# termuxinator/html5-canvas-raytracer

Hardware: AMD Instinct MI355X
Metric: Mpixel/s (higher is better)
Workload: dtype f64; 1 GPU; cfg3: h8 scene (8 spheres, 2 lights, depth 3, supersample 1) at 3840x2160; SCENE, CAMERA AND LAUNCH TABLE RESIDENT (a static frame rendered again and again: cold_frame / new_camera_every_step are the other cases); one launch per frame; kernel=fma

## Files before the change

html5-canvas-raytracer_amd/csrc/rt_kernel.hip:

```cpp

#include <hip/hip_runtime.h>
#include <math.h>
#include <stdint.h>

#include "rt_device.h"
#include "rt_block.h"
#include "rt_wide.h"

#ifndef RT_STRICT
#define RT_STRICT 0
#endif
#if RT_STRICT
#define RT_LAUNCH_NAME rt_launch_trace_strict
#define RT_SCRATCH_NAME rt_scratch_trace_strict
#else
#define RT_LAUNCH_NAME rt_launch_trace_fast
#define RT_SCRATCH_NAME rt_scratch_trace_fast
#endif

#ifndef RT_WAVES_PER_EU
#define RT_WAVES_PER_EU 2
#endif

constexpr unsigned rt_waves_per_eu(bool refract, bool grid, bool w1) {
// ... 28 lines not shown
  [[maybe_unused]] constexpr uint32_t WG_WAVES = W1 ? 1u : RT_WG_THREADS / 64u;
  constexpr uint32_t KT = W1 ? 64u : RT_WG_THREADS;
  extern __shared__ double lds_raw[];
#if defined(RT_WAVE_LOG) && !RT_STRICT
  if (unsigned long long *const wl = rt_cold_args()->wave_log; wl != nullptr && (threadIdx.x & 63u) == 0u) {
    unsigned long long *q = wl + ((size_t)(blockIdx.z * gridDim.x + blockIdx.x) * WG_WAVES + (threadIdx.x >> 6)) * 4u;
    q[0] = __builtin_amdgcn_s_memrealtime();
    q[2] = (unsigned long long)__builtin_amdgcn_s_getreg((4u) | (0u << 6) | (31u << 11)) | ((unsigned long long)__builtin_amdgcn_s_getreg((20u) | (0u << 6) | (31u << 11)) << 32);
    q[3] = rt_entry_index<W1>();
  }
#endif
  const uint32_t tid = threadIdx.x;
  const uint32_t mtl_words = L.n_objects * (uint32_t)(sizeof(rt_mtl) / 8);
  const uint32_t tex_words = 16u * 2u;
  const bool cull_lds_on = (!RT_STRICT && !COUNT) ? !GRID : (L.cull_in_lds != 0u);
  const uint32_t cull_words = cull_lds_on ? L.n_objects * 4u : 0u;
  constexpr bool MTL_ONLY = W1 && !GRID;
  const uint32_t image_words = MTL_ONLY ? mtl_words : mtl_words + tex_words + cull_words;
  constexpr bool IMAGE_IN_LDS = RT_STRICT || COUNT || !(GRID && !REFRACT);
  const uint32_t lds_words = IMAGE_IN_LDS ? image_words : 0u;
  const double *__restrict__ image = (const double *)L.lds_image;
  typedef uint32_t __attribute__((ext_vector_type(4))) rt_u4;
  constexpr uint32_t RT_STAGE_PIECES = 3u;
  const uint32_t image_vec = image_words >> 1;
  [[maybe_unused]] rt_u4 piece[RT_STAGE_PIECES];
  [[maybe_unused]] double stage0 = 0.0;
  const auto stage_issue = [&](const uint32_t tid) __attribute__((always_inline)) {
    if constexpr (!IMAGE_IN_LDS) {
    } else if constexpr (GRID || W1) {
      const rt_u4 *__restrict__ image4 = (const rt_u4 *)L.lds_image;
#pragma unroll
      for (uint32_t i = 0; i < RT_STAGE_PIECES; i++) if (i * KT < image_vec) piece[i] = image4[tid + i * KT];
    } else {
      stage0 = (tid < image_words) ? image[tid] : 0.0;
    }
  };
  constexpr bool UNI_OK = W1 && !REFRACT && !COUNT && !RT_STRICT && !(GRID && SS2);
  if constexpr (!UNI_OK) stage_issue(tid);
  const rt_mtl *mtl = IMAGE_IN_LDS ? (const rt_mtl *)lds_raw : (const rt_mtl *)L.lds_image;
  const rt_texture_desc *tex = (IMAGE_IN_LDS && !MTL_ONLY) ? (const rt_texture_desc *)(lds_raw + mtl_words) : (const rt_texture_desc *)((const double *)L.lds_image + mtl_words);
  const rt_geom *cull_lds = (const rt_geom *)(lds_raw + mtl_words + tex_words);
  double *acc = lds_raw + lds_words + tid;
  rt_geom cull0 = rt_geom{0.0, 0.0, 0.0, 0.0};
  if (!cull_lds_on) { const uint32_t lane0 = tid & 63u; cull0 = L.cull[lane0 < L.n_loop ? lane0 : 0u]; }

  const uint32_t lane = tid & 63u;
  const rt_pixel P0 = rt_pixel_of<SS2, W1>(L, tid);
#if !RT_STRICT
  if constexpr (W1 && !REFRACT && !COUNT && !GRID) rt_head_batch(L);
  if (P0.rows_valid == 0u) return;
#endif
  [[maybe_unused]] bool uni_try = false;
  [[maybe_unused]] uint32_t cell = 0u;
  if constexpr (UNI_OK) {
    uni_try = !P0.sky && (P0.cand >> 16) == 1u;
    if constexpr (!GRID) cell = (P0.cell >> rt_wave_of<W1>(tid)) & 0x11u;
#ifdef RT_TESTING
    if (L.no_uniform) uni_try = false;
    if (L.no_cells) cell = 0u;
#endif
    if (!uni_try && !P0.sky) stage_issue(tid);
  }
  double rgb[3];
  uint32_t cnt[3] = {0u, 0u, 0u};
  if (P0.sky) {
    rgb[0] = L.sky_rgb[0]; rgb[1] = L.sky_rgb[1]; rgb[2] = L.sky_rgb[2];
  } else {
  const uint32_t px = P0.px, frow = P0.frow, sub = P0.sub;
  const uint32_t sx = SS2 ? 2u * px + (sub & 1u) : px;
  const uint32_t sy = SS2 ? 2u * frow + (sub >> 1) : frow;

#if RT_STRICT
  const double d0 = ((double)sx - L.proj_w) + 0.5, d1 = (L.proj_h - (double)sy) - 0.5, d2 = L.proj_d;
#else
  const double d0 = (double)sx + L.ray_bias[0], d1 = L.ray_bias[1] - (double)sy;
#endif
  const v3 o = mk(L.cam_origin[0], L.cam_origin[1], L.cam_origin[2]);
  double rl;
#if RT_STRICT
  const v3 target = mk(o.x + L.cam_axis_x[0] * d0 + L.cam_axis_y[0] * d0 + L.cam_axis_z[0] * d0,
                       o.y + L.cam_axis_x[1] * d1 + L.cam_axis_y[1] * d1 + L.cam_axis_z[1] * d1,
                       o.z + L.cam_axis_x[2] * d2 + L.cam_axis_y[2] * d2 + L.cam_axis_z[2] * d2);
  const v3 ray = unit(mk(target.x - o.x, target.y - o.y, target.z - o.z), &rl);
#else
  const v3 rawray = mk(L.cam_axis_sum[0] * d0, L.cam_axis_sum[1] * d1, L.ray_bias[2]);
  rl = rt_rsqrt_pos(dot(rawray, rawray));
  const v3 ray = mk(rawray.x * rl, rawray.y * rl, rawray.z * rl);
#endif

#ifdef RT_TESTING
  const bool is_probe = L.probe != nullptr && sx == L.probe_x && sy == L.probe_y && blockIdx.z == 0;
#else
  const bool is_probe = false;
#endif
  const auto stage_finish = [&](const uint32_t tid) __attribute__((always_inline)) {
    if constexpr (!IMAGE_IN_LDS) {
    } else if constexpr (GRID || W1) {
      rt_u4 *lds4 = (rt_u4 *)lds_raw;
      const rt_u4 *__restrict__ image4 = (const rt_u4 *)L.lds_image;
#pragma unroll
      for (uint32_t i = 0; i < RT_STAGE_PIECES; i++) {
        const uint32_t k = tid + i * KT;
        if (i * KT < image_vec && k < image_vec) lds4[k] = piece[i];
      }
      for (uint32_t k = tid + RT_STAGE_PIECES * KT; k < image_vec; k += KT) lds4[k] = image4[k];
    } else {
      if (tid < image_words) lds_raw[tid] = stage0;
      for (uint32_t k = tid + RT_WG_THREADS; k < image_words; k += RT_WG_THREADS) lds_raw[k] = image[k];
    }
  };
  [[maybe_unused]] bool uni_done = false;
  if constexpr (UNI_OK) {
    if (uni_try) {
      uni_done = trace_pixel<REFRACT, COUNT, GRID, SS2, false, W1, true>(L, (const rt_mtl *)L.lds_image, (const rt_texture_desc *)((const double *)L.lds_image + mtl_words), acc,
                                                                         cull_lds, cull0, lane, 0.0, 0.0, 0.0, 0.0, o, ray, rgb, cnt, is_probe, P0.cand | (cell << 24));
      if (!uni_done) {
        uint32_t tid4 = threadIdx.x;
        if constexpr (MTL_ONLY) tid4 = rt_lane_again(); else
        asm volatile("" : "+v"(tid4));
        stage_issue(tid4);
        stage_finish(tid4);
      }
#ifdef RT_TESTING
      else if (lane == 0u && L.uniform_waves != nullptr) {
        atomicAdd(L.uniform_waves, 1ull);
        if (cell & 1u) atomicAdd(L.uniform_waves + 1, 1ull);
      }
#endif
    }
  }
  if (!uni_done) {
    if (!UNI_OK || !uni_try) stage_finish(tid);
    if constexpr (IMAGE_IN_LDS) __syncthreads();

    const double bw = SS2 ? 15.0 : 7.0, bh = SS2 ? 3.0 : 7.0;
    const double lx = SS2 ? (double)(2u * ((lane >> 2) & 7u) + (sub & 1u)) : (double)(lane & 7u);
    const double ly = SS2 ? (double)(2u * (lane >> 5) + (sub >> 1)) : (double)(lane >> 3);
    double blk_x0 = 0.0, blk_x1 = 0.0, blk_y0 = 0.0, blk_y1 = 0.0;
    if (!UNI_OK || !uni_try) { blk_x0 = d0 - lx; blk_x1 = blk_x0 + bw; blk_y1 = d1 + ly; blk_y0 = blk_y1 - bh; }
    trace_pixel<REFRACT, COUNT, GRID, SS2, false, W1>(L, mtl, tex, acc, cull_lds, cull0, lane, blk_x0, blk_x1, blk_y0, blk_y1, o, ray, rgb, cnt, is_probe, P0.cand);
  }
  }

  uint32_t tid2 = threadIdx.x;
  if constexpr (W1 && !GRID) tid2 = rt_lane_again(); else
  asm volatile("" : "+v"(tid2));
  const rt_pixel P1 = rt_pixel_of<SS2, W1>(L, tid2);
#if !RT_STRICT
  const uint32_t wide = rt_cold_args()->wide_stores;
  asm volatile("" :: "s"(wide), "s"(L.scatter), "s"(L.rgb24), "s"(L.w), "s"(L.out), "s"(L.frame_stride));
#endif
  const uint32_t frame_i = blockIdx.z;
  const bool valid = P1.valid;
  const uint32_t r8 = to_byte(rgb[0]), g8 = to_byte(rgb[1]), b8 = to_byte(rgb[2]);
#if RT_STRICT
  uint32_t *__restrict__ out = L.scatter ? L.out_frames[frame_i] : L.out + (size_t)frame_i * L.frame_stride;
  const uint32_t orow = L.scatter ? P1.frow : P1.lrow;
#endif
  uint32_t rgbw;
  if (!SS2) rgbw = r8 | (g8 << 8) | (b8 << 16);
  else {
    uint32_t packed = r8 | (g8 << 10) | (b8 << 20);
    packed += __shfl_xor(packed, 1);
    packed += __shfl_xor(packed, 2);
    rgbw = (((packed & 1023u) + 2u) >> 2) | ((((packed >> 10) & 1023u) + 2u) >> 2 << 8) | ((((packed >> 20) & 1023u) + 2u) >> 2 << 16);
  }
#if RT_STRICT
  const uint32_t n_run = 1u;
#else
  const uint32_t n_run = P1.sky ? P1.run : 1u;
#endif
#if defined(RT_ABLATE_STORE) && !RT_STRICT
  asm volatile("" :: "v"(rgbw));
  const bool store_off = ((RT_ABLATE_STORE + 0) == 2 ? P1.sky : true) && rt_cold_args()->n_frames != ~0u;
#endif
#if !RT_STRICT
  if (wide != 0u) {
    const uint32_t lane2 = tid2 & 63u, wave2 = rt_wave_of<W1>(tid2), pix = rgbw | 0xff000000u;
    const uint32_t px0 = P1.px & ~(RT_TILE_W - 1u);
    uint32_t *const band = L.out + (size_t)frame_i * L.frame_stride + (size_t)(P1.lrow - P1.trow) * L.w;
#if defined(RT_ABLATE_STORE)
    if (store_off) {} else
#endif
    if (P1.sky) {
      const rt_wide_piece wp = rt_wide_sky(lane2);
      const rt_px4 v = {pix, pix, pix, pix};
      for (uint32_t t = wave2; t < n_run; t += 4u) {
        const uint32_t px = px0 + t * RT_TILE_W + wp.col;
        if (wp.row < P1.rows_valid && px < L.w) rt_store16(band + (size_t)wp.row * L.w + px, v, (wide & RT_WIDE_THROUGH_SKY) != 0u);
      }
    } else {
      const rt_wide_piece wp = rt_wide_traced(SS2, wave2, lane2);
      const rt_px4 v = {pix, rt_row_down<SS2 ? 4 : 1>(pix), rt_row_down<SS2 ? 8 : 2>(pix), rt_row_down<SS2 ? 12 : 3>(pix)};
      const uint32_t px = px0 + wp.col;
      if (wp.stores && wp.row < P1.rows_valid && px < L.w) rt_store16(band + (size_t)wp.row * L.w + px, v, (wide & RT_WIDE_THROUGH_TRACED) != 0u);
    }
  } else
#endif
  {
#if !RT_STRICT
  uint32_t *__restrict__ out = L.scatter ? L.out_frames[frame_i] : L.out + (size_t)frame_i * L.frame_stride;
  const uint32_t orow = L.scatter ? P1.frow : P1.lrow;
#endif
  if (!W1 && !L.rgb24 && L.scatter && !SS2) {
    uint32_t *tile = (uint32_t *)(lds_raw + lds_words);
    tile[2u * tid2] = rgbw;
// ... 220 lines not shown
```

html5-canvas-raytracer_amd/csrc/rt_kernel_math.h:

```cpp

struct v3 { double x, y, z; };
__device__ __forceinline__ v3 mk(double x, double y, double z) { v3 r; r.x = x; r.y = y; r.z = z; return r; }
__device__ __forceinline__ double dot(const v3 a, const v3 b) { return a.x * b.x + a.y * b.y + a.z * b.z; }

#if RT_STRICT
__device__ __forceinline__ double rt_sqrt(double x) { return sqrt(x); }
template <bool FMIN = false> __device__ __forceinline__ double rt_sqrt_nn(double x) { return sqrt(x); }
__device__ __forceinline__ double rt_rcp(double x) { return 1.0 / x; }
__device__ __forceinline__ double rt_div(double a, double b) { return a / b; }
__device__ __forceinline__ double rt_pow(double x, double e) { return pow(x, e); }
#define RT_DIV_CONST(x, c) ((x) / (c))
__device__ __forceinline__ v3 unit(const v3 v, double *len_out) {
  const double l = sqrt(dot(v, v));
  *len_out = l;
  if (l != 0.0) { const double s = 1.0 / l; return mk(v.x * s, v.y * s, v.z * s); }
  return v;
}
#else
__device__ __forceinline__ double rt_rsqrt_pos(double m) {
  const double y = __builtin_amdgcn_rsq(m);
  const double e = __builtin_fma(-(m * y), y, 1.0);
  return __builtin_fma(0.5 * y, e, y);
}
__device__ __forceinline__ double rt_sqrt(double x) {
  const double y = rt_rsqrt_pos(x);
  double g = x * y;
  g = __builtin_fma(__builtin_fma(-g, g, x), 0.5 * y, g);
  return (x > 0.0) ? g : x;
}
template <bool FMIN = false>
__device__ __forceinline__ double rt_sqrt_nn(double x) {
  double y;
  if constexpr (FMIN) y = __builtin_fmin(__builtin_amdgcn_rsq(x), 1e100);
  else {
    const unsigned long long yb = __builtin_bit_cast(unsigned long long, __builtin_amdgcn_rsq(x));
    const int32_t yh = (int32_t)(yb >> 32);
    y = __builtin_bit_cast(double, ((unsigned long long)(uint32_t)(yh < 0x7fe00000 ? yh : 0x7fe00000) << 32) | (uint32_t)yb);
  }
  const double e = __builtin_fma(-(x * y), y, 1.0);
  y = __builtin_fma(0.5 * y, e, y);
  const double g = x * y;
  return __builtin_fma(__builtin_fma(-g, g, x), 0.5 * y, g);
}
__device__ __forceinline__ double rt_rcp(double x) {
  double y = __builtin_amdgcn_rcp(x);
  y = __builtin_fma(y, __builtin_fma(-x, y, 1.0), y);
  return __builtin_fma(y, __builtin_fma(-x, y, 1.0), y);
}
__device__ __forceinline__ double rt_div(double a, double b) {
  const double r = rt_rcp(b);
  const double q = a * r;
  return __builtin_fma(__builtin_fma(-q, b, a), r, q);
}
#define RT_DIV_CONST(x, c) rt_div_const((x), (c), 1.0 / (c))
__device__ __forceinline__ double rt_div_const(double a, double c, double rc) {
  const double q = a * rc;
  return __builtin_fma(__builtin_fma(-q, c, a), rc, q);
}
__device__ __attribute__((noinline)) double rt_pow_generic(double x, double e) { return pow(x, e); }
template <bool UNI = false, class EP>
__device__ __forceinline__ double rt_pow_spec(double x, int32_t n, EP e) {
  const int32_t n0 = UNI ? n : __builtin_amdgcn_readfirstlane(n);
  if (UNI || __ballot(n != n0) == 0ull) {
    if (n0 < 0) return rt_pow_generic(x, *e);
    uint32_t k = (uint32_t)n0;
    if (k == 0u) return 1.0;
    double b = x;
    uint32_t g = __builtin_ctz(k);
    for (uint32_t i = 0; i < g; i++) b *= b;
    double r = b;
    for (k >>= g + 1u; k != 0u; k >>= g + 1u) {
      g = __builtin_ctz(k);
      for (uint32_t i = 0; i <= g; i++) b *= b;
      r *= b;
    }
    return r;
  }
  if (n < 0) return rt_pow_generic(x, *e);
  double r = 1.0, b = x;
  uint32_t k = (uint32_t)n;
  do { if (k & 1u) r *= b; b *= b; k >>= 1; } while (__ballot(k != 0u) != 0ull);
  return r;
}
__device__ __forceinline__ v3 unit(const v3 v, double *len_out) {
  const double m = dot(v, v);
  const double s = rt_rsqrt_pos(m);
  const bool ok = (m > 0.0);
  *len_out = ok ? m * s : m;
  return ok ? mk(v.x * s, v.y * s, v.z * s) : v;
}
#endif

#if RT_STRICT
#include "rt_fdlibm.h"
template <bool FMIN = false> __device__ __forceinline__ void rt_atan2_asin(double y, double x, double w, double *at, double *as) { *at = fd_atan2(y, x); *as = fd_asin(w); }
#else
__device__ __forceinline__ double rt_fma_k(double a, double b, double k) {
  double r;
  asm("v_fma_f64 %0, %1, %2, %3" : "=v"(r) : "v"(a), "v"(b), "s"(k));
  return r;
}
typedef const double __attribute__((address_space(4))) *rt_trig_kptr;
typedef double __attribute__((ext_vector_type(4))) rt_d4;
#define RT_TRIG_AHEAD 2u
__constant__ unsigned long long RT_TRIG_BITS[32] = {
    0x3eeba404b5e68a13ull, 0xbf23e260bd3237f4ull, 0x3f4b2bb069efb384ull, 0xbf67952daf56de9bull,
    0x3f7d6d43a595c56full, 0xbf8c6ea4a57d9582ull, 0x3f967e295f08b19full, 0xbf9e9ae6fc27006aull,
    0x3fa2c15b5711927aull, 0x3fa059859fea6a70ull, 0xbfa59976e82d3ff0ull, 0xbf90a5a378a05eafull,
    0x3fa82d5d6ef28734ull, 0x3f94052137024d6aull, 0xbfaae5ce6a214619ull, 0x3f7ab3a098a70509ull,
    0x3fae1bb48427b883ull, 0x3f88ed60a300c8d2ull, 0xbfb110e48b207f05ull, 0x3f8c6fa84b77012bull,
    0x3fb3b13657b87036ull, 0x3f91c6c111dccb70ull, 0xbfb745d119378e4full, 0x3f96e89f0a0adacfull,
    0x3fbc71c717e1913cull, 0x3f9f1c72c668963full, 0xbfc2492492376b7dull, 0x3fa6db6db41ce4bdull,
    0x3fc99999999952ccull, 0x3fb333333336fd5bull, 0xbfd5555555555523ull, 0x3fc5555555555380ull};
template <bool FMIN = false>
__device__ __forceinline__ void rt_atan2_asin(double y, double x, double w, double *at, double *as) {
  rt_trig_kptr K = (rt_trig_kptr)(const void *)RT_TRIG_BITS;
  asm volatile("" : "+s"(K));
#define RT_TRIG_GROUP(I) (*(const rt_d4 __attribute__((address_space(4))) *)(K + 4 * (I)))
  rt_d4 g[8];
  g[0] = RT_TRIG_GROUP(0); g[1] = RT_TRIG_GROUP(1);
  const double ax = __builtin_fabs(x), ay = __builtin_fabs(y);
  const double hi = __builtin_fmax(ax, ay), lo = __builtin_fmin(ax, ay);
  const double q = rt_div(lo, hi);
  const double z = q * q;
  const double yw = __builtin_fabs(w);
  const double t = __builtin_fma(yw, -0.5, 0.5);
  const bool big = (yw >= 0.5);
  const double r = big ? t : w * w;
  g[2] = RT_TRIG_GROUP(2);
  double p = g[0][0];
  p = rt_fma_k(p, z, g[0][1]); p = rt_fma_k(p, z, g[0][2]); p = rt_fma_k(p, z, g[0][3]);
  g[3] = RT_TRIG_GROUP(3);
  p = rt_fma_k(p, z, g[1][0]); p = rt_fma_k(p, z, g[1][1]); p = rt_fma_k(p, z, g[1][2]); p = rt_fma_k(p, z, g[1][3]);
  double pa = 0.0;
#pragma unroll
// ... 67 lines not shown
```

html5-canvas-raytracer_amd/csrc/rt_kernel_trace.h:

```cpp

#define RT_PIN() asm volatile("")
#define RT_ROOT(TCA, DISC)                                                                    \
        const double thc_ = rt_sqrt_nn<REFRACT>(DISC);                                                 \
        const double t0_ = (TCA) - thc_, t1_ = (TCA) + thc_;                                  \
        const bool in_ = (t0_ < eps);                                                         \
        const double t_ = in_ ? t1_ : t0_;
#define RT_CAND(IDX, TCA, DISC)                                                               \
      if (!((DISC) < 0.0)) {                                                                  \
        RT_PIN();                                                                             \
        RT_ROOT(TCA, DISC)                                                                    \
        const bool closer_ = (t_ < ht) && !(t_ < eps);              \
        ht = closer_ ? t_ : ht;                                                               \
        hcode = closer_ ? ((int)(2u * (IDX)) + (in_ ? 1 : 0)) : hcode;                        \
      }
#define RT_GENERIC(IDX, G)                                                                    \
      {                                                                                       \
        const v3 Lv_ = mk((G).ox - p.x, (G).oy - p.y, (G).oz - p.z);                          \
        const double tca_ = dot(d, Lv_);                                                      \
        const double disc_ = (G).r2 - (dot(Lv_, Lv_) - tca_ * tca_);                          \
        RT_CAND(IDX, tca_, disc_)                                                             \
      }
#define RT_ANCHORED_DISC(G)                                                                   \
        const double tca_ = d.x * (G).ox + d.y * (G).oy + d.z * (G).oz;                       \
        const double disc_ = __builtin_fma(tca_, tca_, -(G).r2);
#define RT_ANCHORED(IDX, G)                                                                   \
      {                                                                                       \
        RT_ANCHORED_DISC(G)                                                                   \
        RT_CAND(IDX, tca_, disc_)                                                             \
      }

#if !RT_STRICT
__device__ __forceinline__ float rt_q_of(float qp, float x, float c, float rp_over_r) {
  const float ic = __builtin_amdgcn_rcpf(fmaxf(c, 1e-30f));
  return fminf(ic * (qp * (6.f * x + rp_over_r) + x + 0.5f * x * x) + x, 1e30f);
}
__device__ __forceinline__ int rt_lvl(int lv) { return lv & 255; }
#define RT_Q_GET(L_) __builtin_bit_cast(float, (uint32_t)(L_) & 0xffff0000u)
__device__ __forceinline__ int rt_q_put(int lv, float q) { return (int)(((uint32_t)lv & 0xffffu) | ((__builtin_bit_cast(uint32_t, q) + 0xffffu) & 0xffff0000u)); }
__device__ __forceinline__ float rt_r_get(int lv) { return __builtin_bit_cast(float, ((uint32_t)lv & 0xff00u) << 15); }
__device__ __forceinline__ int rt_r_put(int lv, float r) { return (int)(((uint32_t)lv & 0xffff00ffu) | ((((__builtin_bit_cast(uint32_t, r) >> 23) + 1u) & 255u) << 8)); }
constexpr float RT_Q_FLAT = 4096.f;
#define RT_Q_OF(QP, T, INVR, C, RP) rt_q_of((QP), (T) * (INVR), (C), (RP) * (INVR))
#else
__device__ __forceinline__ int rt_lvl(int lv) { return lv; }
#endif

#if !RT_STRICT
#define RT_XY_INDEX(XU, XV, FU, FV)                                                                                \
          const unsigned long long su = __builtin_bit_cast(unsigned long long, (XU) + 6442450944.0), sv = __builtin_bit_cast(unsigned long long, (XV) + 6442450944.0);   \
          uint32_t iu = __builtin_amdgcn_alignbit((uint32_t)(su >> 32), (uint32_t)su, 20u) ^ 0x80000000u;        \
          uint32_t iv = __builtin_amdgcn_alignbit((uint32_t)(sv >> 32), (uint32_t)sv, 20u) ^ 0x80000000u;       \
           \
// ... 10 lines not shown
              const float ex = (float)(h.x - K->cam_origin[0]), ey = (float)(h.y - K->cam_origin[1]), ez = (float)(h.z - K->cam_origin[2]);   \
              q_here = RT_Q_OF(0.f, __builtin_sqrtf(ex * ex + ey * ey + ez * ez), (float)m.inv_r, __builtin_fabsf((float)dot(d, n)), 0.f);       \
            }                                                                                                     \
            double tol = (K->mark_flags & RT_MARK_ALL) ? 2.0 : K->flag_tol * (double)fmaxf(1.f, q_here * (1.f / RT_Q_FLAT));   \
                          \
            if ((K->mark_flags & (RT_MARK_WEIGHT | RT_MARK_ALL)) == RT_MARK_WEIGHT) {                              \
              double S_ = map_valid ? acc[0] : 1.0;                                                               \
              if constexpr (FOLD_FORWARD && REFRACT) for (int i_ = 0; i_ < sp; i_++) S_ *= (parked[i_].map_valid ? parked[i_].S : 1.0) * parked[i_].a3;   \
              if (__builtin_fabs(S_) * 510.0 < 0.9) tol = -1.0;                                                    \
            }                                                                                                     \
             \
            const bool zf = !(K->mark_flags & RT_MARK_ZERO);                                                       \
            const bool bu = (zf && (FU) == 0.0 && (XU) == 0.0) || (__builtin_fabs((XU) - __builtin_rint(XU)) >= tol);    \
            const bool bv = (zf && (FV) == 0.0 && (XV) == 0.0) || (__builtin_fabs((XV) - __builtin_rint(XV)) >= tol);    \
            if (!(bu & bv)) {                                                                                      \
              uint32_t t3 = threadIdx.x;                                                                          \
              if constexpr (W1 && !GRID) t3 = rt_lane_again(); else                                               \
              asm volatile("" : "+v"(t3));                                                                        \
              rt_mark_append<SS2>(rt_pixel_of<SS2, W1>(L, t3));                                                        \
            }                                                                                                     \
          }
#endif

#if !RT_STRICT
#define RT_SDISC(G, TC, DISC)                                                                 \
            const double TC = -(sv.x * (G).ox + sv.y * (G).oy + sv.z * (G).oz);               \
            const double DISC = __builtin_fma(TC, TC, -(G).r2);
#define RT_SROOTS(TC, THC, T0, T1) const double T0 = llen - (TC + THC), T1 = llen - (TC - THC);
#else
#define RT_SDISC(G, TC, DISC)                                                                 \
            const v3 Lv_ = mk((G).ox - h.x, (G).oy - h.y, (G).oz - h.z);                      \
            const double TC = dot(sv, Lv_);                                                   \
            const double DISC = (G).r2 - (dot(Lv_, Lv_) - TC * TC);
#define RT_SROOTS(TC, THC, T0, T1) const double T0 = TC - THC, T1 = TC + THC;
#endif
#define RT_SHADOW(J, G)                                                                       \
            {                                                                                 \
              const bool other_ = ((int)(J) != hi);                                           \
              if (COUNT && other_ && !blocked) tests++;                                       \
              RT_SDISC(G, tc_, disc_)                                                         \
              if (other_ && !(disc_ < 0.0) && !blocked) {                                     \
                RT_PIN();                                                                     \
                const double thc_ = rt_sqrt_nn<REFRACT>(disc_);                                        \
                RT_SROOTS(tc_, thc_, t0_, t1_)                                                \
                const double t_ = (t0_ < eps) ? t1_ : t0_;                                    \
                if ((t_ < llen) && !(t_ < eps)) {                                             \
                  RT_PIN();                                                                   \
                  const double oa4_ = objs[J].albedo[4];                                      \
                  if (oa4_ != 0.0) li = rt_div(li, oa4_);    \
                  else { li = 0.0; blocked = true; }                                          \
                }                                                                             \
              }                                                                               \
            }
#define RT_SHADOW_U(J, G)                                                                     \
            {                                                                               \
              RT_SDISC(G, tc_, disc_)                                                       \
              if (((int)(J) != hi) && !(disc_ < 0.0)) {                                     \
                RT_PIN();                                                                   \
                const double thc_ = rt_sqrt_nn<REFRACT>(disc_);                                      \
                RT_SROOTS(tc_, thc_, t0_, t1_)                                              \
                const double t_ = (t0_ < eps) ? t1_ : t0_;                                  \
                if ((t_ < llen) && !(t_ < eps) && li != 0.0) {                              \
                  RT_PIN();                                                                 \
                  const double oa4_ = objs[J].albedo[4];                                    \
                  li = (oa4_ != 0.0) ? rt_div(li, oa4_) : 0.0;                              \
                }                                                                           \
              }                                                                             \
            }

#define RT_CHAIN_END()                                                                                                          \
        if constexpr (SIX_WAVES) {                                                                                              \
          if (map_valid) {                                                                                                      \
            const double S_ = acc[0];                                                                                           \
            _Pragma("unroll")                                                                                                   \
            for (int c = 0; c < 3; c++) ret[c] = rt_max_nn(acc[(4 + c) * 64u], rt_min_nn(acc[(7 + c) * 64u], __builtin_fma(S_, ret[c], acc[(1 + c) * 64u])));   \
          }                                                                                                                     \
        }

template <bool REFRACT, bool COUNT, bool GRID, bool SS2, bool ITEM = false, bool W1 = false, bool UNI = false>
__device__ __forceinline__ bool trace_pixel(const rt_launch &L, const rt_mtl *mtl, const rt_texture_desc *tex,
                                            [[maybe_unused]] double *acc, [[maybe_unused]] const rt_geom *cull_lds, [[maybe_unused]] const rt_geom cull0, [[maybe_unused]] uint32_t lane,
                                            [[maybe_unused]] double blk_x0, [[maybe_unused]] double blk_x1, [[maybe_unused]] double blk_y0,
                                            [[maybe_unused]] double blk_y1, v3 p, v3 d, double rgb[3], uint32_t cnt[3],
                                            [[maybe_unused]] bool is_probe, [[maybe_unused]] uint32_t cand_host,
                                            [[maybe_unused]] uint32_t own_sx = 0u, [[maybe_unused]] uint32_t own_sy = 0u, [[maybe_unused]] uint32_t own_f = 0u) {
  static_assert(!UNI || (W1 && !REFRACT && !COUNT && !ITEM && !RT_STRICT), "uniform-material path: the one-wave-workgroup product kernels");
#ifdef RT_TESTING
  uint32_t probe_n = 0;
  double probe_li = 0.0;
#endif
  const sphere_kptr objs = (sphere_kptr)L.objects;
  const geom_kptr geom = (geom_kptr)L.geom;
  const uint32_t N = L.n_objects, NL = L.n_lights;
  const double eps = L.epsilon;
  const uint32_t NLOOP = L.n_loop;
  const uint32_t enc = L.enclosing;
  const bool cull_lds_on = (!RT_STRICT && !COUNT) ? (!GRID && !W1) : (L.cull_in_lds != 0u);
#if RT_STRICT
  constexpr bool FOLD_FORWARD = false;
#else
  constexpr bool FOLD_FORWARD = true;
#endif
  constexpr bool LEAN = !RT_STRICT && !REFRACT && !COUNT && !ITEM;
  [[maybe_unused]] frame<REFRACT> stack[FOLD_FORWARD ? 1 : RT_MAX_SEGS];
  [[maybe_unused]] park parked[(FOLD_FORWARD && REFRACT) ? RT_MAX_SEGS : 1];
  [[maybe_unused]] int sp = 0;
  [[maybe_unused]] bool map_valid = false;
  int level = 0;
  [[maybe_unused]] uint32_t tree_path = 1u;
#if defined(RT_TESTING) && defined(RT_ABLATE_BOUNCE)
  uint32_t segs_left = L.segs ? 1 : 0;
#else
  uint32_t segs_left = L.segs;
#endif
  double ret[3] = {0.0, 0.0, 0.0};
  constexpr bool SIX_WAVES = FOLD_FORWARD && W1 && !GRID && !REFRACT && !COUNT && !ITEM && !UNI;
  constexpr bool WAVE_NODE = LEAN && !GRID && !UNI;
  [[maybe_unused]] uint32_t turn = 0u;

  double ht = RT_INF; int hcode = -1;
  if constexpr (UNI) { if (segs_left == 0) return false; }
  if (segs_left != 0) {
        [[maybe_unused]] const geom_kptr ga = (geom_kptr)L.geom_cam;
#if !RT_STRICT
        if constexpr (UNI) {
          const uint32_t i = cand_host & 255u;
          const rt_geom g0 = rt_load_geom32(ga, i);
          typename rt_mtl_src<true>::type &mu = *rt_mtl_at<true>(mtl, i);
          if ((mu.albedo[3] > 0.0 && segs_left > 1) || rt_mtl_kind(mu) == RT_SAMPLER_STARS) return false;
          RT_ANCHORED_DISC(g0)
          const double t0_ = tca_ - rt_sqrt_nn<REFRACT>(disc_);
          const bool met_ = !(disc_ < 0.0) && (t0_ < ht) && !(t0_ < eps);
          if (__ballot(!met_) != 0ull) return false;
#if defined(RT_TESTING) && defined(RT_ABLATE_UNIFORM)
          rgb[0] = rgb[1] = rgb[2] = 0.0;
          return true;
#endif
          ht = t0_; hcode = (int)(2u * i);
        } else
        if (cand_host != 0u) {
          { const uint32_t i = cand_host & 255u; const rt_geom g0 = rt_load_geom32(ga, i); RT_ANCHORED(i, g0) }
          if (cand_host >= (2u << 16)) { const uint32_t i = (cand_host >> 8) & 255u; const rt_geom g0 = rt_load_geom32(ga, i); RT_ANCHORED(i, g0) }
        } else
#endif
        for (uint32_t base = 0; base < NLOOP; base += 64u) {
          const uint32_t j = base + lane;
          const uint32_t jj = j < NLOOP ? j : 0u;
          double c0 = cull0.ox, c1 = cull0.oy, c2 = cull0.oz, c3 = cull0.r2;
          if constexpr (ITEM) {
          } else if (cull_lds_on) {
            const rt_geom __attribute__((address_space(3))) *g = (const rt_geom __attribute__((address_space(3))) *)cull_lds + jj;
            c0 = g->ox; c1 = g->oy; c2 = g->oz; c3 = g->r2;
          } else if (base != 0u || (W1 && !GRID)) {
            const rt_geom __attribute__((address_space(1))) *g = (const rt_geom __attribute__((address_space(1))) *)L.cull + jj;
            c0 = g->ox; c1 = g->oy; c2 = g->oz; c3 = g->r2;
          }
// ... 223 lines not shown
          col[0] = RT_DIV_CONST((double)(texel & 255u), 255.0); col[1] = RT_DIV_CONST((double)((texel >> 8) & 255u), 255.0);
          col[2] = RT_DIV_CONST((double)((texel >> 16) & 255u), 255.0);
        } else if (kind == RT_SAMPLER_CHECKER) {
          if constexpr (!UNI) rt_atan2_asin<REFRACT>(-n.y, -n.x, -n.z, &t_at, &t_as);
          const double u = RT_DIV_CONST(t_at, M_PI) / 2.0 + 0.5;
          const double v = RT_DIV_CONST(t_as, M_PI / 2.0) / 2.0 + 0.5;
          const double xu = u * m.c[6], xv = v * m.c[7];
          RT_XY_INDEX(xu, xv, m.c[6], m.c[7])
          const int c = (int)((iu ^ iv) & 1u);
          if constexpr (UNI) {
            double k0 = m.c[0], k1 = m.c[1], k2 = m.c[2], k3 = m.c[3], k4 = m.c[4], k5 = m.c[5];
            asm volatile("" : "+s"(k0), "+s"(k1), "+s"(k2), "+s"(k3), "+s"(k4), "+s"(k5));
            col[0] = c ? k3 : k0; col[1] = c ? k4 : k1; col[2] = c ? k5 : k2;
          } else { col[0] = m.c[3 * c]; col[1] = m.c[3 * c + 1]; col[2] = m.c[3 * c + 2]; }
#endif
        } else if (!UNI && kind == RT_SAMPLER_STARS) {
          uint32_t sx = own_sx, sy = own_sy, f = own_f;
          if constexpr (!ITEM) {
            f = blockIdx.z;
            uint32_t t3 = threadIdx.x;
            if constexpr (W1 && !GRID) t3 = rt_lane_again(); else
            asm volatile("" : "+v"(t3));
            const rt_pixel P = rt_pixel_of<SS2, W1>(L, t3);
            sx = SS2 ? 2u * P.px + (P.sub & 1u) : P.px; sy = SS2 ? 2u * P.frow + (P.sub >> 1) : P.frow;
          }
          const unsigned long long pix = (unsigned long long)sy * (SS2 ? 2u * L.w : L.w) + sx;
          const uint32_t path = REFRACT ? tree_path : (1u << rt_lvl(level));
          const rt_launch __attribute__((address_space(4))) *K = rt_cold_args();
          const uint32_t mix = lowbias32(K->stars_seed + K->stars_step * f);
          double c = star_uniform((uint32_t)pix, (uint32_t)(pix >> 32), path, mix);
          c = (c >= m.c[6]) ? 0.0 : c * m.c[7];
          col[0] = col[1] = col[2] = c;
        } else { col[0] = m.c[0]; col[1] = m.c[1]; col[2] = m.c[2]; }
#if !RT_STRICT
        }
#endif

        if constexpr (FOLD_FORWARD && REFRACT) {
#pragma unroll
          for (int c = 0; c < 3; c++) acc[(10 + c) * RT_WG_THREADS] = col[c];
        }

        double diffuse = 0.0, specular = 0.0;
        [[maybe_unused]] double draw = 0.0, sraw = 0.0;
#if defined(RT_TESTING) && defined(RT_ABLATE_LIGHT)
        if (false) {
#else
        if (a1 > 0.0 || a2 > 0.0) {
#endif
          double li = RT_COLD(light_intensity);
#if !RT_STRICT
          [[maybe_unused]] uint32_t smask = ~0u;
          if constexpr (!COUNT) { if (primary_node) smask = rt_entry_shadow_masks<W1>(L); }
#endif
          for (uint32_t k = 0; k < NL; k++) {
            double llen;
            const double *lk = (const double *)((const char *)&L.lights[0][0] + (uint32_t)(k * 24u));
#if !RT_STRICT
            [[maybe_unused]] rt_geom_pair gp_first;
            if constexpr (!GRID && !COUNT) {
              [[maybe_unused]] const geom_kptr gl = (geom_kptr)L.geom_light;
              gp_first = rt_load_geom_pair32(gl, k * L.n_objects);
            }
#endif
            const v3 sraw = mk(lk[0] - h.x, lk[1] - h.y, lk[2] - h.z);
            const double lmag = dot(sraw, sraw);
#if RT_STRICT
            const v3 sv = unit(sraw, &llen);
#else
            const double inv_llen = rt_rsqrt_pos(lmag);
            llen = lmag * inv_llen;
            const v3 sv = mk(sraw.x * inv_llen, sraw.y * inv_llen, sraw.z * inv_llen);
#endif
            const double sdot = dot(sv, l);
#if RT_STRICT
            if (sdot <= 0.0) continue;
#else
            if (!(sdot > 0.0)) continue;
#endif
            if (COUNT) cnt[1]++;
            uint32_t tests = 0;
            bool blocked = false;
#if !RT_STRICT
            const geom_kptr gl = (geom_kptr)L.geom_light;
            const uint32_t glo = k * L.n_objects;
#else
            const geom_kptr gl = geom;
            const uint32_t glo = 0u;
#endif
#if defined(RT_TESTING) && defined(RT_ABLATE_SHADOW)
            const uint32_t NS = 0;
#elif defined(RT_TESTING) && defined(RT_ABLATE_SHADOW4)
            const uint32_t NS = NLOOP > 4u ? NLOOP - 4u : NLOOP;
#else
            const uint32_t NS = NLOOP;
#endif
#if !RT_STRICT
            bool no_occluder = false;
            if constexpr (!COUNT) no_occluder = primary_node && k < 2u && ((smask >> (16u * k)) & 0xffffu) == 0u;
            if (no_occluder) {
            } else
            if (GRID && rt_cold_args()->shadow_grid != nullptr && li != 0.0) {
              const void *const sgrid = rt_cold_args()->shadow_grid;
              const double __attribute__((address_space(4))) *gh = (const double __attribute__((address_space(4))) *)sgrid + 16u * k;
              const v3 vv = mk(-sraw.x, -sraw.y, -sraw.z);
              const double vx = gh[0] * vv.x + gh[1] * vv.y + gh[2] * vv.z, vy = gh[3] * vv.x + gh[4] * vv.y + gh[5] * vv.z;
              const double vz = gh[6] * vv.x + gh[7] * vv.y + gh[8] * vv.z;
              const double iz = rt_rcp(vz);
              const double fx = __builtin_fmin(__builtin_fmax((vx * iz - gh[9]) * gh[11], 0.0), (double)(RT_SGRID - 1));
              const double fy = __builtin_fmin(__builtin_fmax((vy * iz - gh[10]) * gh[12], 0.0), (double)(RT_SGRID - 1));
              const bool proj = (vz > 0.0) && (fx == fx) && (fy == fy);
              const uint32_t cell = proj ? (uint32_t)fy * RT_SGRID + (uint32_t)fx : (uint32_t)(RT_SGRID * RT_SGRID);
              const uint32_t words = (NLOOP + 63u) >> 6;
              const uint32_t cells_at = 16u * NL + k * (RT_SGRID * RT_SGRID + 1u) * words;
              for (uint32_t wd = 0; wd < words; wd++) {
                unsigned long long cand = 0ull, todo = __ballot(true);
                while (todo) {
                  const uint32_t c0 = (uint32_t)__builtin_amdgcn_readlane((int)cell, (int)__builtin_ctzll(todo));
                  cand |= rt_load_word32(sgrid, cells_at + c0 * words + wd);
                  todo &= ~__ballot(cell == c0);
                }
                while (cand) {
                  const uint32_t j = (wd << 6) + (uint32_t)__builtin_ctzll(cand);
                  cand &= cand - 1ull;
                  const rt_geom g0 = rt_load_geom32(gl, glo + j);
                  RT_SHADOW_U(j, g0)
                }
              }
            } else
#endif
            if (!COUNT) {
              if constexpr (UNI) RT_PIN();
              if (li != 0.0) {
                uint32_t j = 0;
#if !RT_STRICT
                [[maybe_unused]] uint32_t mk = ~0u;
                if constexpr (!GRID) { if (primary_node && k < 2u) mk = (smask >> (16u * k)) | 0xffff0000u; }
                if constexpr (!GRID) {
                  if (NS >= 2u) { if (mk & 3u) { const rt_geom g0 = gp_first.a, g1 = gp_first.b; RT_SHADOW_U(0u, g0) RT_SHADOW_U(1u, g1) } j = 2u; }
                }
#endif
                for (; j + 2 <= NS; j += 2) {
#if !RT_STRICT
                  if constexpr (WAVE_NODE) { if (((mk >> (j < 30u ? j : 30u)) & 3u) == 0u) continue; } else
                  if (!GRID && j < 31u && ((mk >> j) & 3u) == 0u) continue;
#endif
                  const rt_geom_pair gp = rt_load_geom_pair32(gl, glo + j);
                  const rt_geom g0 = gp.a, g1 = gp.b;
                  RT_SHADOW_U(j, g0) RT_SHADOW_U(j + 1, g1)
                }
#if !RT_STRICT
                if (j < NS && (GRID || j >= 32u || ((mk >> j) & 1u))) { const rt_geom g0 = rt_load_geom32(gl, glo + j); RT_SHADOW_U(j, g0) }
#else
                if (j < NS) { const rt_geom g0 = rt_load_geom32(gl, glo + j); RT_SHADOW_U(j, g0) }
#endif
              }
            } else
            if (COUNT || li != 0.0) {
              uint32_t j = 0;
              for (; j + 2 <= NS; j += 2) {
                const rt_geom g0 = rt_load_geom32(gl, glo + j), g1 = rt_load_geom32(gl, glo + j + 1);
                RT_SHADOW(j, g0) RT_SHADOW(j + 1, g1)
                if (blocked) break;
              }
              if (j < NS && !blocked) { const rt_geom g0 = rt_load_geom32(gl, glo + j); RT_SHADOW(j, g0) }
            }
            if (COUNT) cnt[2] += tests;
            if (li == 0.0) continue;
#if RT_STRICT
            diffuse += li * sdot / lmag;
#else
            diffuse += (li * sdot) * (inv_llen * inv_llen);
#endif
#if defined(RT_TESTING) && defined(RT_ABLATE_SPEC)
            if (false) {
#else
            if (a2 > 0.0) {
#endif
#if RT_STRICT
              double ql;
              const v3 q = unit(reflect(mk(-sv.x, -sv.y, -sv.z), l), &ql);
              const double spd = d.x * -q.x + d.y * -q.y + d.z * -q.z;
#else
              const double t2 = 2.0 * sdot;
              const v3 q = mk(__builtin_fma(l.x, t2, -sv.x), __builtin_fma(l.y, t2, -sv.y), __builtin_fma(l.z, t2, -sv.z));
              const double spd = -(d.x * q.x + d.y * q.y + d.z * q.z);
#endif
#if !RT_STRICT
              typename rt_mtl_src<UNI>::type *spec_m = &m;
              if constexpr (GRID && !REFRACT && !COUNT && !UNI) {
                uint32_t off_ = (uint32_t)hi * (uint32_t)sizeof(rt_mtl);
                asm volatile("" : "+v"(off_));
                spec_m = (const rt_mtl *)((const char *)mtl + off_);
              }
              const int32_t spec_n = spec_m->spec_n;
              if (spd > 0.0) specular += rt_pow_spec<UNI>(spd, spec_n, &spec_m->specular_exponent);
#else
              if (spd > 0.0) specular += rt_pow(spd, m.specular_exponent);
#endif
            }
          }
          if constexpr (UNI) {
            draw = diffuse; sraw = specular;
            diffuse = rt_min1_nn(diffuse) * a1;
            specular = rt_min1_nn(specular) * a2;
          } else {
          diffuse = min1(diffuse) * a1;
          specular = min1(specular) * a2;
          }
#ifdef RT_TESTING
          probe_li = li;
#endif
        }

        if constexpr (SIX_WAVES) {
          uint32_t hi2 = (uint32_t)hi;
          asm volatile("" : "+v"(hi2));
          const rt_mtl &m2 = *rt_mtl_at<false>(mtl, hi2);
          a0 = m2.albedo[0]; a3 = m2.albedo[3];
        }

#if RT_STRICT
        const v3 nq = n;
#else
        const v3 nq = inside ? mk(-l.x, -l.y, -l.z) : l;
#endif
        v3 r = mk(0, 0, 0); double rlen = 0.0;
#if !RT_STRICT
        if constexpr (LEAN) { if (!UNI && a3 > 0.0 && segs_left > 1) r = unit_go(reflect(d, l), &rlen); } else
#endif
        if (!UNI && a3 > 0.0 && segs_left > 1) r = unit(reflect(d, nq), &rlen);
        v3 f = mk(0, 0, 0); double flen = 0.0;
        if (REFRACT && a4 > 0.0 && segs_left > 1) {
          const double dn = dot(d, nq);
          double cosi = -((dn < -1.0) ? -1.0 : min1(dn));
          v3 nn = nq; double eta;
          if (cosi < 0.0) { cosi = -cosi; nn = mk(-nq.x, -nq.y, -nq.z); eta = m.refract_index; }
          else eta = rt_rcp(m.refract_index);
          const double k = 1.0 - eta * eta * (1.0 - cosi * cosi);
          if (k > 0.0) {
            const double q = eta * cosi - rt_sqrt(k);
            f = mk(d.x * eta + nn.x * q, d.y * eta + nn.y * q, d.z * eta + nn.z * q);
          } else f = reflect(d, nn);
          f = unit(f, &flen);
        }

        if constexpr (FOLD_FORWARD && REFRACT) {
#pragma unroll
          for (int c = 0; c < 3; c++) col[c] = acc[(10 + c) * RT_WG_THREADS];
// ... 195 lines not shown
```

Measured before the change: 171,400 Mpixel/s.

## Keep wave-uniform flags and shadow masks in scalar registers, ladder spec pow

Packs the per-wave sky and uniform-try decisions into one flag word pinned to scalar registers. The sky colour is now filled in at store time, so the sky and uniform paths branch on scalar conditions instead of vector masks. In the uniform, non-grid, single-wave path, shadow occluder masks and the albedo nonzero test also go through scalar values, and the specular integer power uses an unrolled compile-time ladder instead of a gap loop. The aim is fewer VCC/exec-mask branches and fewer VGPRs; in exchange the code is larger and relies on inline-asm pinning, and a census script is added to count branch types in the assembly listing.

```diff
diff --git a/html5-canvas-raytracer_amd/csrc/rt_kernel.hip b/html5-canvas-raytracer_amd/csrc/rt_kernel.hip
--- a/html5-canvas-raytracer_amd/csrc/rt_kernel.hip
+++ b/html5-canvas-raytracer_amd/csrc/rt_kernel.hip
@@ -104,6 +104,23 @@
 #endif
   [[maybe_unused]] bool uni_try = false;
   [[maybe_unused]] uint32_t cell = 0u;
+  constexpr bool WAVE_FLAGS = UNI_OK && !GRID;
+  [[maybe_unused]] uint32_t wf = 0u;
+  if constexpr (WAVE_FLAGS) {
+    cell = (P0.cell >> rt_wave_of<W1>(tid)) & 0x11u;
+#ifdef RT_TESTING
+    if (L.no_cells) cell = 0u;
+#endif
+    if (P0.sky) wf = 2u;
+    else {
+      if ((P0.cand >> 16) == 1u) wf = 1u;
+#ifdef RT_TESTING
+      if (L.no_uniform) wf = 0u;
+#endif
+      if ((wf & 1u) == 0u) stage_issue(tid);
+    }
+    asm volatile("" : "+s"(wf));
+  } else
   if constexpr (UNI_OK) {
     uni_try = !P0.sky && (P0.cand >> 16) == 1u;
     if constexpr (!GRID) cell = (P0.cell >> rt_wave_of<W1>(tid)) & 0x11u;
@@ -113,11 +130,13 @@
 #endif
     if (!uni_try && !P0.sky) stage_issue(tid);
   }
+  const auto wf_bit0 = [&]() __attribute__((always_inline)) { uint32_t w_ = wf; asm volatile("" : "+s"(w_)); return (w_ & 1u) != 0u; };
+#define RT_UNI_TRY() (WAVE_FLAGS ? wf_bit0() : uni_try)
   double rgb[3];
   uint32_t cnt[3] = {0u, 0u, 0u};
-  if (P0.sky) {
+  if (!WAVE_FLAGS && P0.sky) {
     rgb[0] = L.sky_rgb[0]; rgb[1] = L.sky_rgb[1]; rgb[2] = L.sky_rgb[2];
-  } else {
+  } else if (!WAVE_FLAGS || (wf & 2u) == 0u) {
   const uint32_t px = P0.px, frow = P0.frow, sub = P0.sub;
   const uint32_t sx = SS2 ? 2u * px + (sub & 1u) : px;
   const uint32_t sy = SS2 ? 2u * frow + (sub >> 1) : frow;
@@ -163,7 +182,7 @@
   };
   [[maybe_unused]] bool uni_done = false;
   if constexpr (UNI_OK) {
-    if (uni_try) {
+    if (RT_UNI_TRY()) {
       uni_done = trace_pixel<REFRACT, COUNT, GRID, SS2, false, W1, true>(L, (const rt_mtl *)L.lds_image, (const rt_texture_desc *)((const double *)L.lds_image + mtl_words), acc,
                                                                          cull_lds, cull0, lane, 0.0, 0.0, 0.0, 0.0, o, ray, rgb, cnt, is_probe, P0.cand | (cell << 24));
       if (!uni_done) {
@@ -182,17 +201,18 @@
     }
   }
   if (!uni_done) {
-    if (!UNI_OK || !uni_try) stage_finish(tid);
+    if (!UNI_OK || !RT_UNI_TRY()) stage_finish(tid);
     if constexpr (IMAGE_IN_LDS) __syncthreads();
 
     const double bw = SS2 ? 15.0 : 7.0, bh = SS2 ? 3.0 : 7.0;
     const double lx = SS2 ? (double)(2u * ((lane >> 2) & 7u) + (sub & 1u)) : (double)(lane & 7u);
     const double ly = SS2 ? (double)(2u * (lane >> 5) + (sub >> 1)) : (double)(lane >> 3);
     double blk_x0 = 0.0, blk_x1 = 0.0, blk_y0 = 0.0, blk_y1 = 0.0;
-    if (!UNI_OK || !uni_try) { blk_x0 = d0 - lx; blk_x1 = blk_x0 + bw; blk_y1 = d1 + ly; blk_y0 = blk_y1 - bh; }
+    if (!UNI_OK || !RT_UNI_TRY()) { blk_x0 = d0 - lx; blk_x1 = blk_x0 + bw; blk_y1 = d1 + ly; blk_y0 = blk_y1 - bh; }
     trace_pixel<REFRACT, COUNT, GRID, SS2, false, W1>(L, mtl, tex, acc, cull_lds, cull0, lane, blk_x0, blk_x1, blk_y0, blk_y1, o, ray, rgb, cnt, is_probe, P0.cand);
   }
   }
+#undef RT_UNI_TRY
 
   uint32_t tid2 = threadIdx.x;
   if constexpr (W1 && !GRID) tid2 = rt_lane_again(); else
@@ -204,6 +224,7 @@
 #endif
   const uint32_t frame_i = blockIdx.z;
   const bool valid = P1.valid;
+  if constexpr (WAVE_FLAGS) { if (P1.sky) { rgb[0] = L.sky_rgb[0]; rgb[1] = L.sky_rgb[1]; rgb[2] = L.sky_rgb[2]; } }
   const uint32_t r8 = to_byte(rgb[0]), g8 = to_byte(rgb[1]), b8 = to_byte(rgb[2]);
 #if RT_STRICT
   uint32_t *__restrict__ out = L.scatter ? L.out_frames[frame_i] : L.out + (size_t)frame_i * L.frame_stride;
diff --git a/html5-canvas-raytracer_amd/csrc/rt_kernel_math.h b/html5-canvas-raytracer_amd/csrc/rt_kernel_math.h
--- a/html5-canvas-raytracer_amd/csrc/rt_kernel_math.h
+++ b/html5-canvas-raytracer_amd/csrc/rt_kernel_math.h
@@ -58,29 +58,21 @@
   return __builtin_fma(__builtin_fma(-q, c, a), rc, q);
 }
 __device__ __attribute__((noinline)) double rt_pow_generic(double x, double e) { return pow(x, e); }
-template <bool UNI = false, class EP>
+#include "rt_spec_walk.h"
+#define RT_SPEC_LADDER 9
+template <bool UNI = false, bool LADDER = false, class EP>
 __device__ __forceinline__ double rt_pow_spec(double x, int32_t n, EP e) {
+  const auto mul = [](double a, double b) __attribute__((always_inline)) { return a * b; };
   const int32_t n0 = UNI ? n : __builtin_amdgcn_readfirstlane(n);
   if (UNI || __ballot(n != n0) == 0ull) {
     if (n0 < 0) return rt_pow_generic(x, *e);
-    uint32_t k = (uint32_t)n0;
+    const uint32_t k = (uint32_t)n0;
     if (k == 0u) return 1.0;
-    double b = x;
-    uint32_t g = __builtin_ctz(k);
-    for (uint32_t i = 0; i < g; i++) b *= b;
-    double r = b;
-    for (k >>= g + 1u; k != 0u; k >>= g + 1u) {
-      g = __builtin_ctz(k);
-      for (uint32_t i = 0; i <= g; i++) b *= b;
-      r *= b;
-    }
-    return r;
+    if constexpr (LADDER) return rt_spec_walk_ladder<RT_SPEC_LADDER>(k, x, mul);
+    else return rt_spec_walk_gaps(k, x, mul);
   }
   if (n < 0) return rt_pow_generic(x, *e);
-  double r = 1.0, b = x;
-  uint32_t k = (uint32_t)n;
-  do { if (k & 1u) r *= b; b *= b; k >>= 1; } while (__ballot(k != 0u) != 0ull);
-  return r;
+  return rt_spec_walk_lanes((uint32_t)n, x, mul, [](bool more) __attribute__((always_inline)) { return __ballot(more) != 0ull; });
 }
 __device__ __forceinline__ v3 unit(const v3 v, double *len_out) {
   const double m = dot(v, v);
diff --git a/html5-canvas-raytracer_amd/csrc/rt_kernel_trace.h b/html5-canvas-raytracer_amd/csrc/rt_kernel_trace.h
--- a/html5-canvas-raytracer_amd/csrc/rt_kernel_trace.h
+++ b/html5-canvas-raytracer_amd/csrc/rt_kernel_trace.h
@@ -1,3 +1,5 @@
+
+#include "rt_uniform_pred.h"
 
 #define RT_PIN() asm volatile("")
 #define RT_ROOT(TCA, DISC)                                                                    \
@@ -114,6 +116,12 @@
                 }                                                                             \
               }                                                                               \
             }
+__device__ __forceinline__ bool rt_nonzero_scalar(double x) {
+  unsigned long long b_ = __builtin_bit_cast(unsigned long long, x);
+  asm volatile("" : "+s"(b_));
+  return rt_nonzero_bits(b_);
+}
+#define RT_OA4_NONZERO(X) (SIX_FORMS ? rt_nonzero_scalar(X) : ((X) != 0.0))
 #define RT_SHADOW_U(J, G)                                                                     \
             {                                                                               \
               RT_SDISC(G, tc_, disc_)                                                       \
@@ -125,7 +133,7 @@
                 if ((t_ < llen) && !(t_ < eps) && li != 0.0) {                              \
                   RT_PIN();                                                                 \
                   const double oa4_ = objs[J].albedo[4];                                    \
-                  li = (oa4_ != 0.0) ? rt_div(li, oa4_) : 0.0;                              \
+                  li = RT_OA4_NONZERO(oa4_) ? rt_div(li, oa4_) : 0.0;                       \
                 }                                                                           \
               }                                                                             \
             }
@@ -164,6 +172,7 @@
   constexpr bool FOLD_FORWARD = true;
 #endif
   constexpr bool LEAN = !RT_STRICT && !REFRACT && !COUNT && !ITEM;
+  [[maybe_unused]] constexpr bool SIX_FORMS = LEAN && W1 && !GRID;
   [[maybe_unused]] frame<REFRACT> stack[FOLD_FORWARD ? 1 : RT_MAX_SEGS];
   [[maybe_unused]] park parked[(FOLD_FORWARD && REFRACT) ? RT_MAX_SEGS : 1];
   [[maybe_unused]] int sp = 0;
@@ -493,6 +502,7 @@
 #if !RT_STRICT
           [[maybe_unused]] uint32_t smask = ~0u;
           if constexpr (!COUNT) { if (primary_node) smask = rt_entry_shadow_masks<W1>(L); }
+          [[maybe_unused]] const unsigned long long smask64 = 0xffffffff00000000ull | smask;
 #endif
           for (uint32_t k = 0; k < NL; k++) {
             double llen;
@@ -538,6 +548,12 @@
 #endif
 #if !RT_STRICT
             bool no_occluder = false;
+            [[maybe_unused]] uint32_t occ = ~0u;
+            if constexpr (SIX_FORMS) {
+              occ = (uint32_t)(smask64 >> (16u * (k < 2u ? k : 2u)));
+              if constexpr (UNI) asm volatile("" : "+s"(occ));
+              no_occluder = (occ & 0xffffu) == 0u;
+            } else
             if constexpr (!COUNT) no_occluder = primary_node && k < 2u && ((smask >> (16u * k)) & 0xffffu) == 0u;
             if (no_occluder) {
             } else
@@ -576,6 +592,8 @@
                 uint32_t j = 0;
 #if !RT_STRICT
                 [[maybe_unused]] uint32_t mk = ~0u;
+                if constexpr (SIX_FORMS) mk = occ | 0xffff0000u;
+                else
                 if constexpr (!GRID) { if (primary_node && k < 2u) mk = (smask >> (16u * k)) | 0xffff0000u; }
                 if constexpr (!GRID) {
                   if (NS >= 2u) { if (mk & 3u) { const rt_geom g0 = gp_first.a, g1 = gp_first.b; RT_SHADOW_U(0u, g0) RT_SHADOW_U(1u, g1) } j = 2u; }
@@ -583,7 +601,7 @@
 #endif
                 for (; j + 2 <= NS; j += 2) {
 #if !RT_STRICT
-                  if constexpr (WAVE_NODE) { if (((mk >> (j < 30u ? j : 30u)) & 3u) == 0u) continue; } else
+                  if constexpr (WAVE_NODE || (UNI && !GRID)) { if (((mk >> (j < 30u ? j : 30u)) & 3u) == 0u) continue; } else
                   if (!GRID && j < 31u && ((mk >> j) & 3u) == 0u) continue;
 #endif
                   const rt_geom_pair gp = rt_load_geom_pair32(gl, glo + j);
@@ -635,7 +653,7 @@
                 spec_m = (const rt_mtl *)((const char *)mtl + off_);
               }
               const int32_t spec_n = spec_m->spec_n;
-              if (spd > 0.0) specular += rt_pow_spec<UNI>(spd, spec_n, &spec_m->specular_exponent);
+              if (spd > 0.0) specular += rt_pow_spec<UNI, SIX_FORMS>(spd, spec_n, &spec_m->specular_exponent);
 #else
               if (spd > 0.0) specular += rt_pow(spd, m.specular_exponent);
 #endif
diff --git a/html5-canvas-raytracer_amd/csrc/rt_spec_walk.h b/html5-canvas-raytracer_amd/csrc/rt_spec_walk.h
--- /dev/null
+++ b/html5-canvas-raytracer_amd/csrc/rt_spec_walk.h
@@ -0,0 +1,64 @@
+#ifndef RT_SPEC_WALK_H
+#define RT_SPEC_WALK_H
+
+#include <stdint.h>
+
+#ifndef RT_SPEC_WALK_FN
+#if defined(__HIPCC__)
+#define RT_SPEC_WALK_FN __device__ __forceinline__
+#else
+#define RT_SPEC_WALK_FN static inline
+#endif
+#endif
+
+template <class MUL>
+RT_SPEC_WALK_FN double rt_spec_walk_gaps(uint32_t k, double x, MUL mul) {
+  double b = x;
+  uint32_t g = (uint32_t)__builtin_ctz(k);
+  for (uint32_t i = 0; i < g; i++) b = mul(b, b);
+  double r = b;
+  for (k >>= g + 1u; k != 0u; k >>= g + 1u) {
+    g = (uint32_t)__builtin_ctz(k);
+    for (uint32_t i = 0; i <= g; i++) b = mul(b, b);
+    r = mul(r, b);
+  }
+  return r;
+}
+
+#define RT_SPEC_WALK_PIN() asm volatile("")
+template <int LEFT, class MUL>
+RT_SPEC_WALK_FN void rt_spec_walk_step(uint32_t k, double &b, double &r, MUL mul) {
+  if constexpr (LEFT > 0) {
+    k >>= 1;
+    if (k != 0u) {
+      RT_SPEC_WALK_PIN();
+      b = mul(b, b);
+      if (k & 1u) { RT_SPEC_WALK_PIN(); r = mul(r, b); }
+      rt_spec_walk_step<LEFT - 1>(k, b, r, mul);
+    }
+  } else {
+    for (k >>= 1; k != 0u; k >>= 1) {
+      b = mul(b, b);
+      if (k & 1u) { RT_SPEC_WALK_PIN(); r = mul(r, b); }
+    }
+  }
+}
+template <int LADDER, class MUL>
+RT_SPEC_WALK_FN double rt_spec_walk_ladder(uint32_t k, double x, MUL mul) {
+  double b = x;
+  const uint32_t g = (uint32_t)__builtin_ctz(k);
+  for (uint32_t i = 0; i < g; i++) b = mul(b, b);
+  k >>= g;
+  double r = b;
+  rt_spec_walk_step<LADDER>(k, b, r, mul);
+  return r;
+}
+
+template <class MUL, class ANY>
+RT_SPEC_WALK_FN double rt_spec_walk_lanes(uint32_t k, double x, MUL mul, ANY any) {
+  double r = 1.0, b = x;
+  do { if (k & 1u) r = mul(r, b); b = mul(b, b); k >>= 1; } while (any(k != 0u));
+  return r;
+}
+
+#endif
diff --git a/html5-canvas-raytracer_amd/csrc/rt_uniform_pred.h b/html5-canvas-raytracer_amd/csrc/rt_uniform_pred.h
--- /dev/null
+++ b/html5-canvas-raytracer_amd/csrc/rt_uniform_pred.h
@@ -0,0 +1,16 @@
+#ifndef RT_UNIFORM_PRED_H
+#define RT_UNIFORM_PRED_H
+
+#include <stdint.h>
+
+#ifndef RT_UNIFORM_PRED_FN
+#if defined(__HIPCC__)
+#define RT_UNIFORM_PRED_FN __device__ __forceinline__
+#else
+#define RT_UNIFORM_PRED_FN static inline
+#endif
+#endif
+
+RT_UNIFORM_PRED_FN bool rt_nonzero_bits(uint64_t bits) { return (bits << 1) != 0u; }
+
+#endif
diff --git a/profiles/uniform_branch_census.py b/profiles/uniform_branch_census.py
--- /dev/null
+++ b/profiles/uniform_branch_census.py
@@ -0,0 +1,96 @@
+#!/usr/bin/env python3
+import argparse
+import json
+import re
+import sys
+
+KERNEL = re.compile(r'^(?:[0-9a-f]+ <)?(_Z\w+|[A-Za-z_]\w*)>?:\s*(;.*)?$')
+VREG = re.compile(r'\bv(\d+|\[\d+:\d+\])')
+CSELECT = re.compile(r'^s_cselect_b64\s+\S+,\s*-1,\s*0$')
+VCC_AND = re.compile(r'^s_andn?2?_b64\s+vcc,\s*exec,\s*\S+$')
+WRITES_VCC = re.compile(r'^(?:[sv]_\w+\s+vcc\b|v_cmp\w*_e32\b|v_(?:addc?|subb?(?:rev)?)_co_u32_e32\b|v_div_scale_\w+\s+\S+,\s*vcc\b)')
+
+
+def census(path):
+    out = {}
+    cur = None
+    files = {}
+    loc = None
+    vcc_from_mask = False
+    for no, raw in enumerate(open(path), 1):
+        line = raw.split(';')[0].split('//')[0].rstrip()
+        s = line.strip()
+        if not s:
+            continue
+        m = KERNEL.match(line)
+        if m and not line.startswith(('\t', ' ', '.')):
+            name = m.group(1)
+            cur = out.setdefault(name, {'cselect': [], 'vcc_branch': [], 'scalar_cmp': [], 'all_vcc_branches': 0, 'all_scc_branches': 0, 'instructions': 0})
+            loc = None
+            vcc_from_mask = False
+            continue
+        if s.startswith('.file'):
+            f = re.match(r'\.file\s+(\d+)\s+(?:"([^"]*)"\s+)?"([^"]*)"', s)
+            if f:
+                files[f.group(1)] = f.group(3)
+            continue
+        if s.startswith('.loc'):
+            f = s.split()
+            if len(f) >= 3:
+                loc = '%s:%s' % (files.get(f[1], f[1]).split('/')[-1], f[2])
+            continue
+        if s.startswith('.Lfunc_end'):
+            cur = None
+            continue
+        if cur is None or s.startswith('.') or s.endswith(':'):
+            continue
+        cur['instructions'] += 1
+        rec = (no, loc, s)
+        if CSELECT.match(s):
+            cur['cselect'].append(rec)
+        if s.startswith('s_cbranch_vcc'):
+            cur['all_vcc_branches'] += 1
+            if vcc_from_mask:
+                cur['vcc_branch'].append(rec)
+        elif s.startswith('s_cbranch_scc'):
+            cur['all_scc_branches'] += 1
+        if s.startswith('v_cmp') and not s.startswith('v_cmpx'):
+            ops = s.split(None, 1)[1] if ' ' in s else ''
+            srcs = ops.split(',')[0 if s.split()[0].endswith('_e32') else 1:]
+            if srcs and not any(VREG.search(o) for o in srcs):
+                cur['scalar_cmp'].append(rec)
+        if VCC_AND.match(s):
+            vcc_from_mask = True
+        elif WRITES_VCC.match(s):
+            vcc_from_mask = False
+    return {k: v for k, v in out.items() if v['instructions']}
+
+
+def counts(c):
+    return {k: (len(v) if isinstance(v, list) else v) for k, v in c.items()}
+
+
+def main():
+    ap = argparse.ArgumentParser(description=__doc__.split('\n')[0])
+    ap.add_argument('listing')
+    ap.add_argument('--kernel', default='', help='only kernels whose (mangled) name contains this')
+    ap.add_argument('--list', action='store_true', help='every counted instruction')
+    ap.add_argument('--json', action='store_true')
+    a = ap.parse_args()
+    res = {k: v for k, v in census(a.listing).items() if a.kernel in k}
+    if a.json:
+        json.dump({k: counts(v) for k, v in res.items()}, sys.stdout, indent=1)
+        print()
+        return
+    for k, v in res.items():
+        c = counts(v)
+        print('%s\n  instructions %d  cselect %d  vcc_branch %d (of %d s_cbranch_vcc*)  scalar_cmp %d  s_cbranch_scc* %d' % (
+            k, c['instructions'], c['cselect'], c['vcc_branch'], c['all_vcc_branches'], c['scalar_cmp'], c['all_scc_branches']))
+        if a.list:
+            for key in ('cselect', 'vcc_branch', 'scalar_cmp'):
+                for no, loc, s in v[key]:
+                    print('    %-10s %6d  %-28s %s' % (key, no, loc or '-', s))
+
+
+if __name__ == '__main__':
+    main()
```

Measured after the change: 178,800 Mpixel/s (median of 6 runs). +4.3%, better.
